# microsoft/GenerativeImage2Text

Hardware: AMD Instinct MI355X
Metric: captions/sec whole-node (GIT_BASE 224px bs=64/GPU greedy len=20) (higher is better)
Workload: dtype f16; 1 GPU; GIT_BASE 224px bs=64/GPU greedy max_len=20 frames=1; global_batch=64, parallelism=dp1, decode_steps_per_caption=19, seq_len_returned=20, hip_graph=True, contexts_in_flight=4, layernorm_folded=True, library=libgitmi_f16.so, encoder_chains=2, schedule=mixed

## Files before the change

### generativeimage2text_amd/csrc/kernels_attn_decode.hip

```cpp
#include "gitmi_common.h"
#include "launchers.h"
#include <algorithm>

namespace gitmi {

static constexpr int HD = 64;

__global__ __launch_bounds__(256) void kv_repack_frag_kernel(const bf16_t* __restrict__ qkv, bf16_t* __restrict__ kf,
                                                             bf16_t* __restrict__ vt, int N, int Np, int H, int d) {
    __shared__ bf16_t vs[32][HD + 8];
    const int s = blockIdx.x, h = blockIdx.y, b = blockIdx.z, tid = threadIdx.x;
    const int nsteps = Np >> 5;
    bf16_t* kdst = kf + ((size_t)b * H + h) * Np * HD;
    bf16_t* vdst = vt + ((size_t)b * H + h) * Np * HD;
    const int key = tid >> 3, ch = tid & 7;
    const int n = s * 32 + key;
    u32x4_t kv = {0u, 0u, 0u, 0u}, vv = kv;
    if (n < N) {
        const bf16_t* src = qkv + ((size_t)b * N + n) * 3 * d + d + h * HD + ch * 8;
        kv = *reinterpret_cast<const u32x4_t*>(src);
        vv = *reinterpret_cast<const u32x4_t*>(src + d);
    }
    *reinterpret_cast<u32x4_t*>(kdst + frag_tile(n >> 4, ch >> 2, 2, (ch & 3) * 16 + (n & 15))) = kv;
    *reinterpret_cast<u32x4_t*>(&vs[key][ch * 8]) = vv;
    __syncthreads();
    const int dt = tid >> 6, lane = tid & 63, lg = lane >> 4, dim = dt * 16 + (lane & 15);
    bf16_t o[8];
#pragma unroll
    for (int e = 0; e < 8; ++e) o[e] = vs[(e >> 2) * 16 + lg * 4 + (e & 3)][dim];
    u32x4_t ov;
#pragma unroll
    for (int e = 0; e < 4; ++e) ov[e] = (uint32_t)o[2 * e] | ((uint32_t)o[2 * e + 1] << 16);
    *reinterpret_cast<u32x4_t*>(vdst + (((size_t)s * 4 + dt) * 64 + lane) * 8) = ov;
}

__device__ __forceinline__ void ld8bf(const bf16_t* p, float (&v)[8]) {
    const u32x4_t r = *reinterpret_cast<const u32x4_t*>(p);
#pragma unroll
    for (int i = 0; i < 4; ++i) {
        unpack2op(r[i], v[2 * i], v[2 * i + 1]);
    }
}

constexpr int ACS = 4;

template <int KB, int TI = 3, int PW = 1, int NH = 2, bool LOOP = false, bool RAGGED = false>
__global__ __launch_bounds__(64 * NH * PW) void attn_decode_mfma_kernel(AttnDecodeArgs a) {
#pragma clang fp contract(off)
    __shared__ float part[PW][NH][KB][HD + 2];
    constexpr int PT = 64 * NH;

    const int tid = threadIdx.x, lane = tid & 63, wave = tid >> 6;
    const int l15 = lane & 15, lg = lane >> 4;
    const int hp = wave / NH, half = wave % NH;
    const int H = a.d / HD;
    const int k = a.beams;
    const bf16_t* QKV = reinterpret_cast<const bf16_t*>(a.qkv);
    bf16_t* TK = reinterpret_cast<bf16_t*>(a.txt_k);
    bf16_t* TV = reinterpret_cast<bf16_t*>(a.txt_v);
    bf16_t* O = reinterpret_cast<bf16_t*>(a.out);
    const int ld3 = 3 * a.d;
    const int Np = a.N_pad, nsteps = Np >> 5;
    const int reps = LOOP ? a.pairs_per_wave : 1;
    auto pair_of = [&](int r) {
        if constexpr (NH == 2) return (int)(blockIdx.y * H + blockIdx.x);
        else return ((int)blockIdx.x * reps + r) * PW + hp;
    };
    struct PairKV { const bf16_t* Kf; const bf16_t* Vt; int nimg_steps, n_img; };
    auto kv_of = [&](int pair) {
        const bool on = PW == 1 || pair < a.n_pairs;
        const int h = on ? pair % H : 0, b = on ? pair / H : 0;
        const int bi = a.img_of ? a.img_of[b] : b;
        PairKV r;
        r.Kf = reinterpret_cast<const bf16_t*>(a.img_k) + ((size_t)bi * H + h) * Np * HD;
        r.Vt = reinterpret_cast<const bf16_t*>(a.img_v) + ((size_t)bi * H + h) * Np * HD;
        r.n_img = RAGGED ? a.ntok[bi] : a.N_img;
        r.nimg_steps = (!on || (a.dbg & 1)) ? 0 : RAGGED ? (r.n_img + 31) >> 5 : nsteps;
        return r;
    };

    bf16x8_t kq[ACS][2][2], vq[ACS][4];
    auto load_chunk = [&](const PairKV& p, int s0) {
#pragma unroll
        for (int c = 0; c < ACS; ++c) {
            const int s = s0 + NH * c;
            const bool on = s < p.nimg_steps && !(a.dbg & 8);
            const bf16_t* kp = p.Kf + frag_tile(2 * s, 0, 2, lane);
            const bf16_t* vp = p.Vt + ((size_t)s * 4 * 64 + lane) * 8;
#pragma unroll
            for (int t = 0; t < 2; ++t)
#pragma unroll
                for (int ds = 0; ds < 2; ++ds) {
                    const bf16x8_t* q = reinterpret_cast<const bf16x8_t*>(kp + (t * 2 + ds) * 512);
                    kq[c][t][ds] = !on ? bf16x8_t{0, 0, 0, 0, 0, 0, 0, 0} : (a.dbg & 16) ? *q : __builtin_nontemporal_load(q);
                }
#pragma unroll
            for (int dt = 0; dt < 4; ++dt) {
                const bf16x8_t* q = reinterpret_cast<const bf16x8_t*>(vp + dt * 512);
                vq[c][dt] = !on ? bf16x8_t{0, 0, 0, 0, 0, 0, 0, 0} : (a.dbg & 16) ? *q : __builtin_nontemporal_load(q);
            }
        }
    };
    PairKV cur = kv_of(pair_of(0));
    load_chunk(cur, half);

  for (int rep = 0; rep < reps; ++rep) {
    const int pair = pair_of(rep);
    const bool head_on = PW == 1 || pair < a.n_pairs;
    const int h = head_on ? pair % H : 0, b = head_on ? pair / H : 0;
    const int row0 = b * k;
    const int nimg_steps = cur.nimg_steps, n_img = cur.n_img;
    if constexpr (LOOP) {
        if (rep > 0 && (a.dbg & 32)) load_chunk(cur, half);
    }

    const int grp = (tid % PT) >> 3, sub = tid & 7;
    const int nt = a.pos + 1;
    int t_j[TI], t_s[TI];
    u32x4_t tkr[TI], tvr[TI];
#pragma unroll
    for (int u = 0; u < TI; ++u) {
        const int it = grp + 8 * NH * u;
        t_j[u] = (head_on && it < k * nt) ? it / nt : -1;
        t_s[u] = it < k * nt ? it % nt : 0;
        tkr[u] = u32x4_t{0u, 0u, 0u, 0u};
        tvr[u] = tkr[u];
        if (t_j[u] >= 0) {
            if (t_s[u] == a.pos) {
                const bf16_t* src = QKV + (size_t)(row0 + t_j[u]) * ld3 + a.d + h * HD + sub * 8;
                tkr[u] = *reinterpret_cast<const u32x4_t*>(src);
                tvr[u] = *reinterpret_cast<const u32x4_t*>(src + a.d);
            } else {
                const int srow = KB == 1 ? row0 : a.kv_src[(size_t)(row0 + t_j[u]) * a.ld_src + t_s[u]];
                const size_t off = ((size_t)srow * a.T_max + t_s[u]) * a.d + h * HD + sub * 8;
                tkr[u] = *reinterpret_cast<const u32x4_t*>(TK + off);
                tvr[u] = *reinterpret_cast<const u32x4_t*>(TV + off);
            }
        }
    }
    if (head_on && (tid % PT) < k * 8) {
        const int j = (tid % PT) >> 3;
        const bf16_t* src = QKV + (size_t)(row0 + j) * ld3 + a.d + h * HD + sub * 8;
        const size_t dst = ((size_t)(row0 + j) * a.T_max + a.pos) * a.d + h * HD + sub * 8;
        *reinterpret_cast<u32x4_t*>(TK + dst) = *reinterpret_cast<const u32x4_t*>(src);
        *reinterpret_cast<u32x4_t*>(TV + dst) = *reinterpret_cast<const u32x4_t*>(src + a.d);
    }

    bf16x8_t qf[2];
#pragma unroll
    for (int ds = 0; ds < 2; ++ds) {
        float qv[8] = {0.f, 0.f, 0.f, 0.f, 0.f, 0.f, 0.f, 0.f};
        if (head_on && l15 < k) ld8bf(QKV + (size_t)(row0 + l15) * ld3 + h * HD + ds * 32 + lg * 8, qv);
        u32x4_t t;
#pragma unroll
        for (int e = 0; e < 4; ++e) t[e] = pack2bf(qv[2 * e] * a.scale, qv[2 * e + 1] * a.scale);
        qf[ds] = __builtin_bit_cast(bf16x8_t, t);
    }
    float m_i = -INFINITY, l_i = 0.f;
    f32x4_t oacc[4];
#pragma unroll
    for (int dt = 0; dt < 4; ++dt) oacc[dt] = f32x4_t{0.f, 0.f, 0.f, 0.f};

    for (int s0 = half; s0 < nimg_steps; s0 += NH * ACS) {
        if (s0 != half) load_chunk(cur, s0);
        f32x4_t sc[ACS][2];
        float cm = -INFINITY;
#pragma unroll
        for (int c = 0; c < ACS; ++c) {
            const int s = s0 + NH * c;
#pragma unroll
            for (int t = 0; t < 2; ++t) {
                sc[c][t] = mfma16(kq[c][t][0], qf[0], f32x4_t{0.f, 0.f, 0.f, 0.f});
                sc[c][t] = mfma16(kq[c][t][1], qf[1], sc[c][t]);
            }
#pragma unroll
            for (int t = 0; t < 2; ++t)
#pragma unroll
                for (int r = 0; r < 4; ++r) {
                    if (s * 32 + t * 16 + lg * 4 + r >= (RAGGED ? n_img : a.N_img) || s >= nimg_steps) sc[c][t][r] = -INFINITY;
                    cm = fmaxf(cm, sc[c][t][r]);
                }
        }
        cm = fmaxf(cm, __shfl_xor(cm, 16, 64));
        cm = fmaxf(cm, __shfl_xor(cm, 32, 64));
        const float mn = fmaxf(m_i, cm);
        if (s0 != half) {
            const float al = fast_exp(m_i - mn);
            l_i *= al;
#pragma unroll
            for (int dt = 0; dt < 4; ++dt) { oacc[dt][0] *= al; oacc[dt][1] *= al; oacc[dt][2] *= al; oacc[dt][3] *= al; }
        }
        m_i = mn;
#pragma unroll
        for (int c = 0; c < ACS; ++c) {
            float p[8];
#pragma unroll
            for (int t = 0; t < 2; ++t)
#pragma unroll
                for (int r = 0; r < 4; ++r) {
                    p[t * 4 + r] = fast_exp(sc[c][t][r] - mn);
                    l_i += p[t * 4 + r];
                }
            u32x4_t pp;
#pragma unroll
            for (int e = 0; e < 4; ++e) pp[e] = pack2bf(p[2 * e], p[2 * e + 1]);
            const bf16x8_t pf = __builtin_bit_cast(bf16x8_t, pp);
            if (a.dbg & 4) {
#pragma unroll
                for (int dt = 0; dt < 4; ++dt) asm volatile("" ::"v"(vq[c][dt]));
                asm volatile("" ::"v"(pf));
                continue;
            }
#pragma unroll
            for (int dt = 0; dt < 4; ++dt) oacc[dt] = mfma16(vq[c][dt], pf, oacc[dt]);
        }
    }
    l_i += __shfl_xor(l_i, 16, 64);
    l_i += __shfl_xor(l_i, 32, 64);
    float q[KB][8], m[KB], l[KB], o[KB][8];
#pragma unroll
    for (int j = 0; j < KB; ++j) {
        m[j] = -INFINITY;
        l[j] = 0.f;
#pragma unroll
        for (int e = 0; e < 8; ++e) { q[j][e] = 0.f; o[j][e] = 0.f; }
        if (head_on && j < k) {
            ld8bf(QKV + (size_t)(row0 + j) * ld3 + h * HD + sub * 8, q[j]);
#pragma unroll
            for (int e = 0; e < 8; ++e) q[j][e] *= a.scale;
        }
    }
    auto dot8 = [&](const float (&x)[8], const float (&y)[8]) {
        float p = 0.f;
#pragma unroll
        for (int e = 0; e < 8; ++e) p = fmaf(x[e], y[e], p);
        p += __shfl_xor(p, 1, 64);
        p += __shfl_xor(p, 2, 64);
        p += __shfl_xor(p, 4, 64);
        return p;
    };
    auto text_item = [&](int jj, const float (&kv)[8], const float (&vv)[8]) {
#pragma unroll
        for (int j = 0; j < KB; ++j) {
            if (j == jj) {
                const float sv = dot8(q[j], kv);
                const float mn = fmaxf(m[j], sv);
                const float al = fast_exp(m[j] - mn);
                const float p = fast_exp(sv - mn);
                l[j] = fmaf(l[j], al, p);
#pragma unroll
                for (int e = 0; e < 8; ++e) o[j][e] = fmaf(o[j][e], al, p * vv[e]);
                m[j] = mn;
            }
        }
    };
    auto unpack = [&](const u32x4_t& r, float (&v)[8]) {
#pragma unroll
        for (int i = 0; i < 4; ++i) {
            unpack2op(r[i], v[2 * i], v[2 * i + 1]);
        }
    };
#pragma unroll
    for (int u = 0; u < TI; ++u) {
        if (t_j[u] >= 0 && !(a.dbg & 2)) {
            float kv[8], vv[8];
            unpack(tkr[u], kv);
            unpack(tvr[u], vv);
            text_item(t_j[u], kv, vv);
        }
    }
    if (head_on) {
        for (int it = grp + 8 * NH * TI; it < k * nt; it += 8 * NH) {
            const int j = it / nt, sidx = it % nt;
            float kv[8], vv[8];
            if (sidx == a.pos) {
                ld8bf(QKV + (size_t)(row0 + j) * ld3 + a.d + h * HD + sub * 8, kv);
                ld8bf(QKV + (size_t)(row0 + j) * ld3 + 2 * a.d + h * HD + sub * 8, vv);
            } else {
                const int srow = KB == 1 ? row0 : a.kv_src[(size_t)(row0 + j) * a.ld_src + sidx];
                ld8bf(TK + ((size_t)srow * a.T_max + sidx) * a.d + h * HD + sub * 8, kv);
                ld8bf(TV + ((size_t)srow * a.T_max + sidx) * a.d + h * HD + sub * 8, vv);
            }
            text_item(j, kv, vv);
        }
    }
    if constexpr (LOOP) {
        if (rep + 1 < reps) {
            cur = kv_of(pair_of(rep + 1));
            if (!(a.dbg & 32)) load_chunk(cur, half);
        }
    }
#pragma unroll
    for (int j = 0; j < KB; ++j) {
#pragma unroll
        for (int off = 8; off < 64; off <<= 1) {
            const float m2 = __shfl_xor(m[j], off, 64);
            const float l2 = __shfl_xor(l[j], off, 64);
            const float mn = fmaxf(m[j], m2);
            const float a1 = m[j] == -INFINITY ? 0.f : fast_exp(m[j] - mn);
            const float a2 = m2 == -INFINITY ? 0.f : fast_exp(m2 - mn);
            l[j] = fmaf(l[j], a1, l2 * a2);
#pragma unroll
            for (int e = 0; e < 8; ++e) {
                const float o2 = __shfl_xor(o[j][e], off, 64);
                o[j][e] = fmaf(o[j][e], a1, o2 * a2);
            }
            m[j] = mn;
        }
    }
    if (l15 < k) {
#pragma unroll
        for (int dt = 0; dt < 4; ++dt)
#pragma unroll
            for (int r = 0; r < 4; ++r) part[hp][half][l15][dt * 16 + lg * 4 + r] = oacc[dt][r];
        if (lg == 0) { part[hp][half][l15][HD] = m_i; part[hp][half][l15][HD + 1] = l_i; }
    }
    if constexpr (NH > 1) __syncthreads(); else __builtin_amdgcn_wave_barrier();
#pragma unroll
    for (int j = 0; j < KB; ++j) {
        if (lane < 8 && j < k) {
            const float mi = part[hp][half][j][HD], li = part[hp][half][j][HD + 1];
            const float mn = fmaxf(mi, m[j]);
            const float a1 = mi == -INFINITY ? 0.f : fast_exp(mi - mn);
            const float a2 = m[j] == -INFINITY ? 0.f : fast_exp(m[j] - mn);
#pragma unroll
            for (int e = 0; e < 8; ++e) part[hp][half][j][sub * 8 + e] = fmaf(part[hp][half][j][sub * 8 + e], a1, o[j][e] * a2);
            if (sub == 0) { part[hp][half][j][HD] = mn; part[hp][half][j][HD + 1] = fmaf(li, a1, l[j] * a2); }
        }
    }
    if constexpr (NH > 1) __syncthreads(); else __builtin_amdgcn_wave_barrier();
    if (head_on)
    for (int i = tid % PT; i < k * HD; i += PT) {
        const int j = i / HD, dd = i % HD;
        if constexpr (NH == 1) {
            const float r1 = part[hp][0][j][dd] / part[hp][0][j][HD + 1];
            if (a.out_frag) O[frag_offset(row0 + j, h * HD + dd, a.d >> 5)] = f2bf(r1);
            else O[(size_t)(row0 + j) * a.d + h * HD + dd] = f2bf(r1);
            continue;
        }
        constexpr int H1 = NH - 1;
        const float m0 = part[hp][0][j][HD], m1 = part[hp][H1][j][HD];
        const float mm = fmaxf(m0, m1);
        const float a0 = m0 == -INFINITY ? 0.f : fast_exp(m0 - mm);
        const float a1 = m1 == -INFINITY ? 0.f : fast_exp(m1 - mm);
        const float num = fmaf(a0, part[hp][0][j][dd], a1 * part[hp][H1][j][dd]);
        const float den = fmaf(a0, part[hp][0][j][HD + 1], a1 * part[hp][H1][j][HD + 1]);
        const float r = num / den;
        if (a.out_frag) O[frag_offset(row0 + j, h * HD + dd, a.d >> 5)] = f2bf(r);
        else O[(size_t)(row0 + j) * a.d + h * HD + dd] = f2bf(r);
    }
    if constexpr (NH == 1) __builtin_amdgcn_wave_barrier();
  }
}

typedef __attribute__((address_space(3))) void attn_lds_void_t;

template <int N> __device__ __forceinline__ void attn_wait_vm() { asm volatile("s_waitcnt vmcnt(%0)" ::"n"(N) : "memory"); }
__device__ __forceinline__ void attn_wait_slots_ahead(int ahead) {
    switch (ahead) {
        case 0: attn_wait_vm<0>(); break;
        case 1: attn_wait_vm<4>(); break;
        case 2: attn_wait_vm<8>(); break;
        case 3: attn_wait_vm<12>(); break;
        case 4: attn_wait_vm<16>(); break;
        case 5: attn_wait_vm<20>(); break;
        case 6: attn_wait_vm<24>(); break;
        case 7: attn_wait_vm<28>(); break;
        case 8: attn_wait_vm<32>(); break;
        case 9: attn_wait_vm<36>(); break;
        case 10: attn_wait_vm<40>(); break;
        default: attn_wait_vm<44>(); break;
    }
}

constexpr int AS_WAVES = 4;
constexpr int AS_SLOT = 4096;

template <int KB, int TI, int RING>
__global__ __launch_bounds__(64 * AS_WAVES) void attn_decode_stream_kernel(AttnDecodeArgs a) {
#pragma clang fp contract(off)
    static_assert(RING >= 2 && RING <= 12, "ring depth");
    __shared__ __attribute__((aligned(16))) unsigned char ring_mem[AS_WAVES][RING * AS_SLOT];
    __shared__ float part[AS_WAVES][KB][HD + 2];

    const int tid = threadIdx.x, lane = tid & 63;
    const int wave = __builtin_amdgcn_readfirstlane(tid >> 6);
    const int l15 = lane & 15, lg = lane >> 4;
    const int H = a.d / HD;
    const int k = a.beams;
    const bf16_t* QKV = reinterpret_cast<const bf16_t*>(a.qkv);
    bf16_t* TK = reinterpret_cast<bf16_t*>(a.txt_k);
    bf16_t* TV = reinterpret_cast<bf16_t*>(a.txt_v);
    bf16_t* O = reinterpret_cast<bf16_t*>(a.out);
    const int ld3 = 3 * a.d;
    const int Np = a.N_pad, nsteps = Np >> 5;
    unsigned char* ring = ring_mem[wave];

    const int W = (int)gridDim.x * AS_WAVES, w0 = (int)blockIdx.x * AS_WAVES + wave;
    const int npw = w0 < a.n_pairs ? (a.n_pairs - 1 - w0) / W + 1 : 0;
    const int slots_per_pair = 2 * nsteps;
    const int total_slots = npw * slots_per_pair;

    int issued = 0;
    int p_ord = 0, p_s0 = 0, p_v = 0, p_c = 0;
    const bf16_t* p_K = nullptr; const bf16_t* p_V = nullptr;
    auto producer_pair = [&]() {
        const int pair = w0 + p_ord * W;
        const int h = pair % H, b = pair / H;
        const int bi = a.img_of ? a.img_of[b] : b;
        p_K = reinterpret_cast<const bf16_t*>(a.img_k) + ((size_t)bi * H + h) * Np * HD;
        p_V = reinterpret_cast<const bf16_t*>(a.img_v) + ((size_t)bi * H + h) * Np * HD;
    };
    if (npw > 0) producer_pair();
    auto issue_slot = [&]() {
        if (issued >= total_slots) return;
        const bf16_t* src = (p_v ? p_V : p_K) + (size_t)(p_s0 + p_c) * (AS_SLOT / 2) + lane * 8;
        unsigned char* dst = ring + (issued % RING) * AS_SLOT;
#pragma unroll
        for (int f = 0; f < 4; ++f)
            __builtin_amdgcn_global_load_lds((const void*)(src + f * 512), (attn_lds_void_t*)(dst + f * 1024), 16, 0, 2);
        ++issued;
        const int nsc = min(ACS, nsteps - p_s0);
        if (++p_c == nsc) {
            p_c = 0;
            if (p_v == 0) p_v = 1;
            else {
                p_v = 0; p_s0 += ACS;
                if (p_s0 >= nsteps) { p_s0 = 0; ++p_ord; if (p_ord < npw) producer_pair(); }
            }
        }
    };
    for (int i = 0; i < RING; ++i) issue_slot();

    int consumed = 0;
    auto slot_ready = [&]() -> const unsigned char* {
        const int ahead = issued - consumed - 1;
        if (ahead == RING - 1) attn_wait_vm<4 * (RING - 1)>();
        else attn_wait_slots_ahead(ahead);
        return ring + (consumed % RING) * AS_SLOT;
    };
    auto slot_done = [&]() {
        asm volatile("s_waitcnt lgkmcnt(0)" ::: "memory");
        ++consumed;
        issue_slot();
    };

    for (int ord = 0; ord < npw; ++ord) {
        const int pair = w0 + ord * W;
        const int h = pair % H, b = pair / H;
        const int row0 = b * k;

        const int grp = lane >> 3, sub = lane & 7;
        const int nt = a.pos + 1;
        int t_j[TI], t_s[TI];
        u32x4_t tkr[TI], tvr[TI];
#pragma unroll
        for (int u = 0; u < TI; ++u) {
            const int it = grp + 8 * u;
            t_j[u] = it < k * nt ? it / nt : -1;
            t_s[u] = it < k * nt ? it % nt : 0;
            tkr[u] = u32x4_t{0u, 0u, 0u, 0u};
            tvr[u] = tkr[u];
            if (t_j[u] >= 0) {
                if (t_s[u] == a.pos) {
                    const bf16_t* src = QKV + (size_t)(row0 + t_j[u]) * ld3 + a.d + h * HD + sub * 8;
                    tkr[u] = *reinterpret_cast<const u32x4_t*>(src);
                    tvr[u] = *reinterpret_cast<const u32x4_t*>(src + a.d);
                } else {
                    const int srow = KB == 1 ? row0 : a.kv_src[(size_t)(row0 + t_j[u]) * a.ld_src + t_s[u]];
                    const size_t off = ((size_t)srow * a.T_max + t_s[u]) * a.d + h * HD + sub * 8;
                    tkr[u] = *reinterpret_cast<const u32x4_t*>(TK + off);
                    tvr[u] = *reinterpret_cast<const u32x4_t*>(TV + off);
                }
            }
        }
        if (lane < k * 8) {
            const int j = lane >> 3;
            const bf16_t* src = QKV + (size_t)(row0 + j) * ld3 + a.d + h * HD + sub * 8;
            const size_t dst = ((size_t)(row0 + j) * a.T_max + a.pos) * a.d + h * HD + sub * 8;
            *reinterpret_cast<u32x4_t*>(TK + dst) = *reinterpret_cast<const u32x4_t*>(src);
            *reinterpret_cast<u32x4_t*>(TV + dst) = *reinterpret_cast<const u32x4_t*>(src + a.d);
        }

        bf16x8_t qf[2];
#pragma unroll
        for (int ds = 0; ds < 2; ++ds) {
            float qv[8] = {0.f, 0.f, 0.f, 0.f, 0.f, 0.f, 0.f, 0.f};
            if (l15 < k) ld8bf(QKV + (size_t)(row0 + l15) * ld3 + h * HD + ds * 32 + lg * 8, qv);
            u32x4_t t;
#pragma unroll
            for (int e = 0; e < 4; ++e) t[e] = pack2bf(qv[2 * e] * a.scale, qv[2 * e + 1] * a.scale);
            qf[ds] = __builtin_bit_cast(bf16x8_t, t);
        }
        float m_i = -INFINITY, l_i = 0.f;
        f32x4_t oacc[4];
#pragma unroll
        for (int dt = 0; dt < 4; ++dt) oacc[dt] = f32x4_t{0.f, 0.f, 0.f, 0.f};

        for (int s0 = 0; s0 < nsteps; s0 += ACS) {
            f32x4_t sc[ACS][2];
            float cm = -INFINITY;
#pragma unroll
            for (int c = 0; c < ACS; ++c) {
                const int s = s0 + c;
                if (s < nsteps) {
                    const unsigned char* sl = slot_ready();
                    bf16x8_t kq[2][2];
#pragma unroll
                    for (int t = 0; t < 2; ++t)
#pragma unroll
                        for (int ds = 0; ds < 2; ++ds)
                            kq[t][ds] = *reinterpret_cast<const bf16x8_t*>(sl + (t * 2 + ds) * 1024 + lane * 16);
                    __builtin_amdgcn_sched_barrier(0);
#pragma unroll
                    for (int t = 0; t < 2; ++t) {
                        sc[c][t] = mfma16(kq[t][0], qf[0], f32x4_t{0.f, 0.f, 0.f, 0.f});
                        sc[c][t] = mfma16(kq[t][1], qf[1], sc[c][t]);
                    }
                    slot_done();
                } else {
                    sc[c][0] = f32x4_t{0.f, 0.f, 0.f, 0.f};
                    sc[c][1] = sc[c][0];
                }
#pragma unroll
                for (int t = 0; t < 2; ++t)
#pragma unroll
                    for (int r = 0; r < 4; ++r) {
                        if (s * 32 + t * 16 + lg * 4 + r >= a.N_img || s >= nsteps) sc[c][t][r] = -INFINITY;
                        cm = fmaxf(cm, sc[c][t][r]);
                    }
            }
            cm = fmaxf(cm, __shfl_xor(cm, 16, 64));
            cm = fmaxf(cm, __shfl_xor(cm, 32, 64));
            const float mn = fmaxf(m_i, cm);
            if (s0 != 0) {
                const float al = fast_exp(m_i - mn);
                l_i *= al;
#pragma unroll
                for (int dt = 0; dt < 4; ++dt) { oacc[dt][0] *= al; oacc[dt][1] *= al; oacc[dt][2] *= al; oacc[dt][3] *= al; }
            }
            m_i = mn;
#pragma unroll
            for (int c = 0; c < ACS; ++c) {
                float p[8];
#pragma unroll
                for (int t = 0; t < 2; ++t)
#pragma unroll
                    for (int r = 0; r < 4; ++r) {
                        p[t * 4 + r] = fast_exp(sc[c][t][r] - mn);
                        l_i += p[t * 4 + r];
                    }
                u32x4_t pp;
#pragma unroll
                for (int e = 0; e < 4; ++e) pp[e] = pack2bf(p[2 * e], p[2 * e + 1]);
                const bf16x8_t pf = __builtin_bit_cast(bf16x8_t, pp);
                if (s0 + c < nsteps) {
                    const unsigned char* sl = slot_ready();
                    bf16x8_t vq[4];
#pragma unroll
                    for (int dt = 0; dt < 4; ++dt) vq[dt] = *reinterpret_cast<const bf16x8_t*>(sl + dt * 1024 + lane * 16);
                    __builtin_amdgcn_sched_barrier(0);
#pragma unroll
                    for (int dt = 0; dt < 4; ++dt) oacc[dt] = mfma16(vq[dt], pf, oacc[dt]);
                    slot_done();
                } else {
#pragma unroll
                    for (int dt = 0; dt < 4; ++dt) oacc[dt] = mfma16(bf16x8_t{0, 0, 0, 0, 0, 0, 0, 0}, pf, oacc[dt]);
                }
            }
        }
        l_i += __shfl_xor(l_i, 16, 64);
        l_i += __shfl_xor(l_i, 32, 64);
        float q[KB][8], m[KB], l[KB], o[KB][8];
#pragma unroll
        for (int j = 0; j < KB; ++j) {
            m[j] = -INFINITY;
            l[j] = 0.f;
#pragma unroll
            for (int e = 0; e < 8; ++e) { q[j][e] = 0.f; o[j][e] = 0.f; }
            if (j < k) {
                ld8bf(QKV + (size_t)(row0 + j) * ld3 + h * HD + sub * 8, q[j]);
#pragma unroll
                for (int e = 0; e < 8; ++e) q[j][e] *= a.scale;
            }
        }
        auto dot8 = [&](const float (&x)[8], const float (&y)[8]) {
            float p = 0.f;
#pragma unroll
            for (int e = 0; e < 8; ++e) p = fmaf(x[e], y[e], p);
            p += __shfl_xor(p, 1, 64);
            p += __shfl_xor(p, 2, 64);
            p += __shfl_xor(p, 4, 64);
            return p;
        };
        auto text_item = [&](int jj, const float (&kv)[8], const float (&vv)[8]) {
#pragma unroll
            for (int j = 0; j < KB; ++j) {
                if (j == jj) {
                    const float sv = dot8(q[j], kv);
                    const float mn = fmaxf(m[j], sv);
                    const float al = fast_exp(m[j] - mn);
                    const float p = fast_exp(sv - mn);
                    l[j] = fmaf(l[j], al, p);
#pragma unroll
                    for (int e = 0; e < 8; ++e) o[j][e] = fmaf(o[j][e], al, p * vv[e]);
                    m[j] = mn;
                }
            }
        };
        auto unpack = [&](const u32x4_t& r, float (&v)[8]) {
#pragma unroll
            for (int i = 0; i < 4; ++i) unpack2op(r[i], v[2 * i], v[2 * i + 1]);
        };
#pragma unroll
        for (int u = 0; u < TI; ++u) {
            if (t_j[u] >= 0) {
                float kv[8], vv[8];
                unpack(tkr[u], kv);
                unpack(tvr[u], vv);
                text_item(t_j[u], kv, vv);
            }
        }
        for (int it = grp + 8 * TI; it < k * nt; it += 8) {
            const int j = it / nt, sidx = it % nt;
            float kv[8], vv[8];
            if (sidx == a.pos) {
                ld8bf(QKV + (size_t)(row0 + j) * ld3 + a.d + h * HD + sub * 8, kv);
                ld8bf(QKV + (size_t)(row0 + j) * ld3 + 2 * a.d + h * HD + sub * 8, vv);
            } else {
                const int srow = KB == 1 ? row0 : a.kv_src[(size_t)(row0 + j) * a.ld_src + sidx];
                ld8bf(TK + ((size_t)srow * a.T_max + sidx) * a.d + h * HD + sub * 8, kv);
                ld8bf(TV + ((size_t)srow * a.T_max + sidx) * a.d + h * HD + sub * 8, vv);
            }
            text_item(j, kv, vv);
        }
#pragma unroll
        for (int j = 0; j < KB; ++j) {
#pragma unroll
            for (int off = 8; off < 64; off <<= 1) {
                const float m2 = __shfl_xor(m[j], off, 64);
                const float l2 = __shfl_xor(l[j], off, 64);
                const float mn = fmaxf(m[j], m2);
                const float a1 = m[j] == -INFINITY ? 0.f : fast_exp(m[j] - mn);
                const float a2 = m2 == -INFINITY ? 0.f : fast_exp(m2 - mn);
                l[j] = fmaf(l[j], a1, l2 * a2);
#pragma unroll
                for (int e = 0; e < 8; ++e) {
                    const float o2 = __shfl_xor(o[j][e], off, 64);
                    o[j][e] = fmaf(o[j][e], a1, o2 * a2);
                }
                m[j] = mn;
            }
        }
        if (l15 < k) {
#pragma unroll
            for (int dt = 0; dt < 4; ++dt)
#pragma unroll
                for (int r = 0; r < 4; ++r) part[wave][l15][dt * 16 + lg * 4 + r] = oacc[dt][r];
            if (lg == 0) { part[wave][l15][HD] = m_i; part[wave][l15][HD + 1] = l_i; }
        }
        __builtin_amdgcn_wave_barrier();
#pragma unroll
        for (int j = 0; j < KB; ++j) {
            if (lane < 8 && j < k) {
                const float mi = part[wave][j][HD], li = part[wave][j][HD + 1];
                const float mn = fmaxf(mi, m[j]);
                const float a1 = mi == -INFINITY ? 0.f : fast_exp(mi - mn);
                const float a2 = m[j] == -INFINITY ? 0.f : fast_exp(m[j] - mn);
#pragma unroll
                for (int e = 0; e < 8; ++e) part[wave][j][sub * 8 + e] = fmaf(part[wave][j][sub * 8 + e], a1, o[j][e] * a2);
                if (sub == 0) { part[wave][j][HD] = mn; part[wave][j][HD + 1] = fmaf(li, a1, l[j] * a2); }
            }
        }
        __builtin_amdgcn_wave_barrier();
        for (int i = lane; i < k * HD; i += 64) {
            const int j = i / HD, dd = i % HD;
            const float r1 = part[wave][j][dd] / part[wave][j][HD + 1];
            if (a.out_frag) O[frag_offset(row0 + j, h * HD + dd, a.d >> 5)] = f2bf(r1);
            else O[(size_t)(row0 + j) * a.d + h * HD + dd] = f2bf(r1);
        }
        __builtin_amdgcn_wave_barrier();
    }
}

hipError_t launch_kv_repack_frag(const void* qkv, void* kf, void* vt, int B, int N, int N_pad, int H, int d, hipStream_t s) {
    if (B <= 0 || N <= 0) return hipSuccess;
    if (N_pad % 32 || N_pad < N) return hipErrorInvalidValue;
    hipLaunchKernelGGL(kv_repack_frag_kernel, dim3(N_pad / 32, H, B), dim3(256), 0, s, (const bf16_t*)qkv, (bf16_t*)kf,
                       (bf16_t*)vt, N, N_pad, H, d);
    return hipGetLastError();
}

hipError_t launch_attn_decode_mfma(const AttnDecodeArgs& a, int B, int H, hipStream_t s) {
    if (B <= 0) return hipSuccess;
    if (a.beams > 8 || a.N_pad % 32 || a.N_pad < a.N_img || a.N_img < 1) return hipErrorInvalidValue;
    if (a.ntok && a.stream_wgs > 0) return hipErrorInvalidValue;
    AttnDecodeArgs p = a;
    p.n_pairs = B * H;
    if (a.stream_wgs > 0) {
        const int nwg = std::max(1, std::min(a.stream_wgs, (p.n_pairs + AS_WAVES - 1) / AS_WAVES));
        if (a.beams <= 1) hipLaunchKernelGGL((attn_decode_stream_kernel<1, 3, 9>), dim3(nwg), dim3(64 * AS_WAVES), 0, s, p);
        else if (a.beams <= 2) hipLaunchKernelGGL((attn_decode_stream_kernel<2, 3, 9>), dim3(nwg), dim3(64 * AS_WAVES), 0, s, p);
        else if (a.beams <= 4) hipLaunchKernelGGL((attn_decode_stream_kernel<4, 3, 9>), dim3(nwg), dim3(64 * AS_WAVES), 0, s, p);
        else hipLaunchKernelGGL((attn_decode_stream_kernel<8, 3, 8>), dim3(nwg), dim3(64 * AS_WAVES), 0, s, p);
        return hipGetLastError();
    }
    if (a.ntok) {
        const dim3 grid(H, B);
        if (a.beams <= 1) hipLaunchKernelGGL((attn_decode_mfma_kernel<1, 3, 1, 2, false, true>), grid, dim3(128), 0, s, p);
        else if (a.beams <= 2) hipLaunchKernelGGL((attn_decode_mfma_kernel<2, 3, 1, 2, false, true>), grid, dim3(128), 0, s, p);
        else if (a.beams <= 4) hipLaunchKernelGGL((attn_decode_mfma_kernel<4, 3, 1, 2, false, true>), grid, dim3(128), 0, s, p);
        else hipLaunchKernelGGL((attn_decode_mfma_kernel<8, 3, 1, 2, false, true>), grid, dim3(128), 0, s, p);
        return hipGetLastError();
    }
    const bool one_wave = a.waves_per_pair == 1 || (a.waves_per_pair != 2 && a.N_pad <= 8 * 32);
    if (!one_wave) {
        const dim3 grid(H, B);
        if (a.beams <= 1) hipLaunchKernelGGL((attn_decode_mfma_kernel<1>), grid, dim3(128), 0, s, p);
        else if (a.beams <= 2) hipLaunchKernelGGL((attn_decode_mfma_kernel<2>), grid, dim3(128), 0, s, p);
        else if (a.beams <= 4) hipLaunchKernelGGL((attn_decode_mfma_kernel<4>), grid, dim3(128), 0, s, p);
        else hipLaunchKernelGGL((attn_decode_mfma_kernel<8>), grid, dim3(128), 0, s, p);
        return hipGetLastError();
    }
    int pw = a.pairs_per_wg >= 8 ? 8 : a.pairs_per_wg >= 4 || a.pairs_per_wg <= 0 ? 4 : a.pairs_per_wg >= 2 ? 2 : 1;
    while (pw > 1 && p.n_pairs / pw < 96) pw >>= 1;
    int ppw = pw == 8 && a.pairs_per_wave > 1 ? a.pairs_per_wave : 1;
    while (ppw > 1 && p.n_pairs / (pw * ppw) < 24) --ppw;
    p.pairs_per_wave = ppw;
    const int per_wg = pw * ppw;
#define GITMI_ATTN1(KBV)                                                                                                   \
    do {                                                                                                                   \
        if (pw == 8 && ppw > 1) hipLaunchKernelGGL((attn_decode_mfma_kernel<KBV, 3, 8, 1, true>), dim3((p.n_pairs + per_wg - 1) / per_wg), dim3(512), 0, s, p); \
        else if (pw == 8) hipLaunchKernelGGL((attn_decode_mfma_kernel<KBV, 3, 8, 1>), dim3((p.n_pairs + 7) / 8), dim3(512), 0, s, p); \
        else if (pw == 4) hipLaunchKernelGGL((attn_decode_mfma_kernel<KBV, 3, 4, 1>), dim3((p.n_pairs + 3) / 4), dim3(256), 0, s, p); \
        else if (pw == 2) hipLaunchKernelGGL((attn_decode_mfma_kernel<KBV, 3, 2, 1>), dim3((p.n_pairs + 1) / 2), dim3(128), 0, s, p); \
        else hipLaunchKernelGGL((attn_decode_mfma_kernel<KBV, 3, 1, 1>), dim3(p.n_pairs), dim3(64), 0, s, p);                         \
    } while (0)
    if (a.beams <= 1) GITMI_ATTN1(1);
    else if (a.beams <= 2) GITMI_ATTN1(2);
    else if (a.beams <= 4) GITMI_ATTN1(4);
    else { if (pw == 8) { pw = 4; ppw = 1; p.pairs_per_wave = 1; } GITMI_ATTN1(8); }
#undef GITMI_ATTN1
    return hipGetLastError();
}

}
```

Baseline: 11570 captions/s.

## Handle image-token tail via scalar text path instead of padded MFMA step

The image KV repack now stores the partial final 32-token block in a plain row-major layout, and the decode attention kernels run MFMA only over full 32-token steps. The leftover image tokens (e.g. 197 = 6*32+5) are folded into the per-lane scalar loop that already handles text tokens. This avoids a whole padded MFMA step that was mostly zero-filled. In exchange the scalar item loop gets longer and more branchy, and the repack layout is now split between fragment-tiled and row-major.

```diff
diff --git a/generativeimage2text_amd/csrc/kernels_attn_decode.hip b/generativeimage2text_amd/csrc/kernels_attn_decode.hip
--- a/generativeimage2text_amd/csrc/kernels_attn_decode.hip
+++ b/generativeimage2text_amd/csrc/kernels_attn_decode.hip
@@ -21,6 +21,11 @@
         kv = *reinterpret_cast<const u32x4_t*>(src);
         vv = *reinterpret_cast<const u32x4_t*>(src + d);
     }
+    if (s >= (N >> 5)) {
+        *reinterpret_cast<u32x4_t*>(kdst + (size_t)s * 32 * HD + tid * 8) = kv;
+        *reinterpret_cast<u32x4_t*>(vdst + (size_t)s * 32 * HD + tid * 8) = vv;
+        return;
+    }
     *reinterpret_cast<u32x4_t*>(kdst + frag_tile(n >> 4, ch >> 2, 2, (ch & 3) * 16 + (n & 15))) = kv;
     *reinterpret_cast<u32x4_t*>(&vs[key][ch * 8]) = vv;
     __syncthreads();
@@ -60,13 +65,13 @@
     bf16_t* TV = reinterpret_cast<bf16_t*>(a.txt_v);
     bf16_t* O = reinterpret_cast<bf16_t*>(a.out);
     const int ld3 = 3 * a.d;
-    const int Np = a.N_pad, nsteps = Np >> 5;
+    const int Np = a.N_pad, nfull = a.N_img >> 5;
     const int reps = LOOP ? a.pairs_per_wave : 1;
     auto pair_of = [&](int r) {
         if constexpr (NH == 2) return (int)(blockIdx.y * H + blockIdx.x);
         else return ((int)blockIdx.x * reps + r) * PW + hp;
     };
-    struct PairKV { const bf16_t* Kf; const bf16_t* Vt; int nimg_steps, n_img; };
+    struct PairKV { const bf16_t* Kf; const bf16_t* Vt; int nimg_steps, n_img, n_tail; };
     auto kv_of = [&](int pair) {
         const bool on = PW == 1 || pair < a.n_pairs;
         const int h = on ? pair % H : 0, b = on ? pair / H : 0;
@@ -75,7 +80,9 @@
         r.Kf = reinterpret_cast<const bf16_t*>(a.img_k) + ((size_t)bi * H + h) * Np * HD;
         r.Vt = reinterpret_cast<const bf16_t*>(a.img_v) + ((size_t)bi * H + h) * Np * HD;
         r.n_img = RAGGED ? a.ntok[bi] : a.N_img;
-        r.nimg_steps = (!on || (a.dbg & 1)) ? 0 : RAGGED ? (r.n_img + 31) >> 5 : nsteps;
+        const bool img_on = on && !(a.dbg & 1);
+        r.nimg_steps = !img_on ? 0 : RAGGED ? min((r.n_img + 31) >> 5, nfull) : nfull;
+        r.n_tail = img_on ? max(r.n_img - nfull * 32, 0) : 0;
         return r;
     };
 
@@ -116,23 +123,32 @@
 
     const int grp = (tid % PT) >> 3, sub = tid & 7;
     const int nt = a.pos + 1;
-    int t_j[TI], t_s[TI];
+    const int n_tail = cur.n_tail, n_ti = k * n_tail, n_items = n_ti + k * nt;
+    const bf16_t* tailK = cur.Kf + (size_t)nfull * 32 * HD;
+    const bf16_t* tailV = cur.Vt + (size_t)nfull * 32 * HD;
+    int t_j[TI];
     u32x4_t tkr[TI], tvr[TI];
 #pragma unroll
     for (int u = 0; u < TI; ++u) {
         const int it = grp + 8 * NH * u;
-        t_j[u] = (head_on && it < k * nt) ? it / nt : -1;
-        t_s[u] = it < k * nt ? it % nt : 0;
+        t_j[u] = -1;
         tkr[u] = u32x4_t{0u, 0u, 0u, 0u};
         tvr[u] = tkr[u];
-        if (t_j[u] >= 0) {
-            if (t_s[u] == a.pos) {
+        if (head_on && it < n_ti) {
+            t_j[u] = it / n_tail;
+            const int off = (it % n_tail) * HD + sub * 8;
+            tkr[u] = *reinterpret_cast<const u32x4_t*>(tailK + off);
+            tvr[u] = *reinterpret_cast<const u32x4_t*>(tailV + off);
+        } else if (head_on && it < n_items) {
+            const int ix = it - n_ti, ts = ix % nt;
+            t_j[u] = ix / nt;
+            if (ts == a.pos) {
                 const bf16_t* src = QKV + (size_t)(row0 + t_j[u]) * ld3 + a.d + h * HD + sub * 8;
                 tkr[u] = *reinterpret_cast<const u32x4_t*>(src);
                 tvr[u] = *reinterpret_cast<const u32x4_t*>(src + a.d);
             } else {
-                const int srow = KB == 1 ? row0 : a.kv_src[(size_t)(row0 + t_j[u]) * a.ld_src + t_s[u]];
-                const size_t off = ((size_t)srow * a.T_max + t_s[u]) * a.d + h * HD + sub * 8;
+                const int srow = KB == 1 ? row0 : a.kv_src[(size_t)(row0 + t_j[u]) * a.ld_src + ts];
+                const size_t off = ((size_t)srow * a.T_max + ts) * a.d + h * HD + sub * 8;
                 tkr[u] = *reinterpret_cast<const u32x4_t*>(TK + off);
                 tvr[u] = *reinterpret_cast<const u32x4_t*>(TV + off);
             }
@@ -270,10 +286,15 @@
         }
     }
     if (head_on) {
-        for (int it = grp + 8 * NH * TI; it < k * nt; it += 8 * NH) {
-            const int j = it / nt, sidx = it % nt;
+        for (int it = grp + 8 * NH * TI; it < n_items; it += 8 * NH) {
+            const bool tail = it < n_ti;
+            const int ix = tail ? it : it - n_ti;
+            const int j = tail ? ix / n_tail : ix / nt, sidx = tail ? ix % n_tail : ix % nt;
             float kv[8], vv[8];
-            if (sidx == a.pos) {
+            if (tail) {
+                ld8bf(tailK + sidx * HD + sub * 8, kv);
+                ld8bf(tailV + sidx * HD + sub * 8, vv);
+            } else if (sidx == a.pos) {
                 ld8bf(QKV + (size_t)(row0 + j) * ld3 + a.d + h * HD + sub * 8, kv);
                 ld8bf(QKV + (size_t)(row0 + j) * ld3 + 2 * a.d + h * HD + sub * 8, vv);
             } else {
@@ -393,7 +414,8 @@
     bf16_t* TV = reinterpret_cast<bf16_t*>(a.txt_v);
     bf16_t* O = reinterpret_cast<bf16_t*>(a.out);
     const int ld3 = 3 * a.d;
-    const int Np = a.N_pad, nsteps = Np >> 5;
+    const int Np = a.N_pad, nsteps = a.N_img >> 5;
+    const int n_tail = a.N_img & 31;
     unsigned char* ring = ring_mem[wave];
 
     const int W = (int)gridDim.x * AS_WAVES, w0 = (int)blockIdx.x * AS_WAVES + wave;
@@ -452,23 +474,33 @@
 
         const int grp = lane >> 3, sub = lane & 7;
         const int nt = a.pos + 1;
-        int t_j[TI], t_s[TI];
+        const int n_ti = k * n_tail, n_items = n_ti + k * nt;
+        const int bi = a.img_of ? a.img_of[b] : b;
+        const bf16_t* tailK = reinterpret_cast<const bf16_t*>(a.img_k) + (((size_t)bi * H + h) * Np + (size_t)nsteps * 32) * HD;
+        const bf16_t* tailV = reinterpret_cast<const bf16_t*>(a.img_v) + (((size_t)bi * H + h) * Np + (size_t)nsteps * 32) * HD;
+        int t_j[TI];
         u32x4_t tkr[TI], tvr[TI];
 #pragma unroll
         for (int u = 0; u < TI; ++u) {
             const int it = grp + 8 * u;
-            t_j[u] = it < k * nt ? it / nt : -1;
-            t_s[u] = it < k * nt ? it % nt : 0;
+            t_j[u] = -1;
             tkr[u] = u32x4_t{0u, 0u, 0u, 0u};
             tvr[u] = tkr[u];
-            if (t_j[u] >= 0) {
-                if (t_s[u] == a.pos) {
+            if (it < n_ti) {
+                t_j[u] = it / n_tail;
+                const int off = (it % n_tail) * HD + sub * 8;
+                tkr[u] = *reinterpret_cast<const u32x4_t*>(tailK + off);
+                tvr[u] = *reinterpret_cast<const u32x4_t*>(tailV + off);
+            } else if (it < n_items) {
+                const int ix = it - n_ti, ts = ix % nt;
+                t_j[u] = ix / nt;
+                if (ts == a.pos) {
                     const bf16_t* src = QKV + (size_t)(row0 + t_j[u]) * ld3 + a.d + h * HD + sub * 8;
                     tkr[u] = *reinterpret_cast<const u32x4_t*>(src);
                     tvr[u] = *reinterpret_cast<const u32x4_t*>(src + a.d);
                 } else {
-                    const int srow = KB == 1 ? row0 : a.kv_src[(size_t)(row0 + t_j[u]) * a.ld_src + t_s[u]];
-                    const size_t off = ((size_t)srow * a.T_max + t_s[u]) * a.d + h * HD + sub * 8;
+                    const int srow = KB == 1 ? row0 : a.kv_src[(size_t)(row0 + t_j[u]) * a.ld_src + ts];
+                    const size_t off = ((size_t)srow * a.T_max + ts) * a.d + h * HD + sub * 8;
                     tkr[u] = *reinterpret_cast<const u32x4_t*>(TK + off);
                     tvr[u] = *reinterpret_cast<const u32x4_t*>(TV + off);
                 }
@@ -621,10 +653,15 @@
                 text_item(t_j[u], kv, vv);
             }
         }
-        for (int it = grp + 8 * TI; it < k * nt; it += 8) {
-            const int j = it / nt, sidx = it % nt;
+        for (int it = grp + 8 * TI; it < n_items; it += 8) {
+            const bool tail = it < n_ti;
+            const int ix = tail ? it : it - n_ti;
+            const int j = tail ? ix / n_tail : ix / nt, sidx = tail ? ix % n_tail : ix % nt;
             float kv[8], vv[8];
-            if (sidx == a.pos) {
+            if (tail) {
+                ld8bf(tailK + sidx * HD + sub * 8, kv);
+                ld8bf(tailV + sidx * HD + sub * 8, vv);
+            } else if (sidx == a.pos) {
                 ld8bf(QKV + (size_t)(row0 + j) * ld3 + a.d + h * HD + sub * 8, kv);
                 ld8bf(QKV + (size_t)(row0 + j) * ld3 + 2 * a.d + h * HD + sub * 8, vv);
             } else {
```

Result: no change. 11520 captions/s, median of 3 (-0.4%).
